# learner-shx/SVG-IR

Hardware: AMD Instinct MI355X
Metric: Gaussian-surfels/sec fwd+bwd @800x800 (1 view) (higher is better)
Workload: dtype f32; 1 GPU; cfg2: rgss path, P=200000 surfels, 800x800, SH degree 3, S=5, VS=0, fwd+bwd, one view per step per GPU (BASELINE.json configs[1] = cfg2 at N=1; configs[3] = cfg4, view r on rank r, at N>1); num_rendered=673008, parallelism=view-parallel x1, per_rank_cpus=not pinned

## Files before the change

svg-ir_amd/csrc/api.hip:

```cpp
#include <algorithm>
#include <cstdarg>
#include <cstdio>
#include <atomic>
#include <cstdlib>
#include <ctime>
#include <memory>
#include <mutex>
#include <string>
#include <vector>

#include "common.hpp"
#include "workload_history.hpp"

using namespace svgir;

namespace {

thread_local std::string g_err;
std::atomic<bool> g_prof{false};
WorkloadHistory g_history;
unsigned long long* pinned_words(size_t n) {
    void* ptr = nullptr;
    if (hipHostMalloc(&ptr, n * sizeof(unsigned long long), hipHostMallocCoherent) != hipSuccess) { (void)hipGetLastError(); return nullptr; }
    std::fill_n((unsigned long long*)ptr, n, 0ull);
    return (unsigned long long*)ptr;
}
unsigned long long* g_pinned = nullptr;
std::atomic<uint32_t> g_pinned_tag{0};
constexpr unsigned kPinnedSlots = 256;
std::once_flag g_pinned_once;
std::mutex g_pinned_mu;
uint64_t g_pinned_busy[kPinnedSlots / 64];
struct PinnedSlot {
    unsigned long long* at = nullptr; uint32_t tag = 0; int index = -1;
    PinnedSlot() {
        std::call_once(g_pinned_once, [] { g_pinned = pinned_words(2 * kPinnedSlots); });
        tag = ++g_pinned_tag;
        if (tag == 0) tag = ++g_pinned_tag;
        if (!g_pinned) return;
        static const unsigned usable = [] { const char* e = getenv("SVGIR_PINNED_SLOTS"); return e ? (unsigned)std::min<long>(std::max<long>(atol(e), 0), kPinnedSlots) : kPinnedSlots; }();
        std::lock_guard<std::mutex> lk(g_pinned_mu);
        for (unsigned i = 0; i < usable; i++)
            if (!(g_pinned_busy[i / 64] >> (i % 64) & 1ull)) {
                g_pinned_busy[i / 64] |= 1ull << (i % 64);
                index = (int)i;
                at = g_pinned + 2 * index;
                return;
            }
    }
    ~PinnedSlot() {
        if (index < 0) return;
        std::lock_guard<std::mutex> lk(g_pinned_mu);
        g_pinned_busy[index / 64] &= ~(1ull << (index % 64));
    }
    PinnedSlot(const PinnedSlot&) = delete;
    PinnedSlot& operator=(const PinnedSlot&) = delete;
};
double spin_budget_s() {
    static const double v = [] {
        const char* e = getenv("SVGIR_SPIN_MS");
        return e ? std::max(0.0, atof(e)) * 1e-3 : 0.05;
    }();
    return v;
}
inline bool tagged_pair(volatile unsigned long long* at, uint32_t tag, uint32_t* w0, uint32_t* w1) {
    const unsigned long long v0 = at[0], v1 = at[1];
    if ((uint32_t)(v0 >> 32) != tag || (uint32_t)(v1 >> 32) != tag) return false;
    *w0 = (uint32_t)v0; *w1 = (uint32_t)v1;
    return true;
}
bool pinned_spin(volatile unsigned long long* at, uint32_t tag, uint32_t* w0, uint32_t* w1) {
    struct timespec t0;
    clock_gettime(CLOCK_MONOTONIC, &t0);
    const double budget = spin_budget_s();
    for (long long spin = 0;; spin++) {
        if (tagged_pair(at, tag, w0, w1)) return true;
        if ((spin & 255) == 255 || budget == 0.0) {
            struct timespec t1;
            clock_gettime(CLOCK_MONOTONIC, &t1);
            const double el = (double)(t1.tv_sec - t0.tv_sec) + 1e-9 * (double)(t1.tv_nsec - t0.tv_nsec);
            if (el >= budget) return false;
            if (el > 5e-3) { struct timespec ts = {0, 20000}; nanosleep(&ts, nullptr); }
        }
    }
}
struct ViewEntry { const void* key = nullptr; uint32_t tag = 0; int cap_R = 0; long long cap_slots = -1; unsigned long long stamp = 0;
                   bool queue = false;
                   bool recorded = false;
                   hipStream_t stream = nullptr; };
constexpr int kViewEntries = 1024;
std::mutex g_view_mu;
ViewEntry g_view[kViewEntries];
constexpr int kViewWords = 4;
unsigned long long* g_view_pinned = nullptr;
unsigned long long g_view_clock = 0;
// ... 394 lines not shown
            if (int rc = check("prepass")) return rc;
            if (timed) stage_mark(tm, "prepass");
        }
        if (p->shade) {
            svgir_shade_params sp = p->shade->sp;
            sp.subset = nullptr; sp.subset_count = nullptr;
            if (prepass) {
                uint32_t* cnt = G.shade_work + partition_work_words(P) - 1;
                launch_partition(P, G.needed, nullptr, G.shade_list, G.shade_work, cnt, s);
                sp.subset = G.shade_list; sp.subset_count = cnt;
            } else if (shade_subset) {
                sp.subset = depth_order; sp.subset_count = G.counters + 3;
            }
            if (shade_forward_impl(&sp, p->shade->reduced, const_cast<float*>(p->features), const_cast<float*>(p->vfeatures), true, s) != 0)
                return fail(SVGIR_ERR_INVALID, "fused shading: svgir_shade_forward rejected its parameters");
            if (int rc = check("shade")) return rc;
            if (timed) stage_mark(tm, "shade");
        }
        if (features_ready && hipStreamWaitEvent(s, features_ready, 0) != hipSuccess) return fail(SVGIR_ERR_HIP, "waiting for the features event");
        if (launch_render_fwd(ra, svgss, s) < 0) launch_render_fwd_generic(ra, svgss, s);
        if (int rc = check("render")) return rc;
        if (timed) stage_mark(tm, "render");
        return 0;
    }

    int begin() {
        if (int rc = validate(p, true)) return rc;
        features_ready = (hipEvent_t)p->features_ready;
        if (!o || !c.geom || !c.binning || !c.image) return fail(SVGIR_ERR_INVALID, "outputs / allocators must be provided");
        P = p->P; v = view_grid(p->W, p->H);
        svgss = p->variant == SVGIR_SVGSS;
        if (P == 0) {
            const size_t N = (size_t)v.W * v.H;
            HIP_OK(hipMemsetAsync(o->out_color, 0, 3 * N * 4, s));
            HIP_OK(hipMemsetAsync(o->out_normal, 0, 3 * N * 4, s));
            HIP_OK(hipMemsetAsync(o->out_depth, 0, N * 4, s));
            HIP_OK(hipMemsetAsync(o->out_opacity, 0, N * 4, s));
            if (p->S) HIP_OK(hipMemsetAsync(o->out_feature, 0, (size_t)p->S * N * 4, s));
            if (svgss && p->VS) HIP_OK(hipMemsetAsync(o->out_vfeature, 0, (size_t)(p->VS / 4) * N * 4, s));
            if (!svgss && o->out_pseudo_normal) HIP_OK(hipMemsetAsync(o->out_pseudo_normal, 0, 3 * N * 4, s));
            if (!svgss && o->out_surface_xyz) HIP_OK(hipMemsetAsync(o->out_surface_xyz, 0, 3 * N * 4, s));
            done = true;
            return 1;
        }
        gblob = c.geom(geom_layout(nullptr, P).bytes, c.geom_ctx);
        iblob = c.image(image_layout(nullptr, v.W, v.H).bytes, c.image_ctx);
        if (!gblob || !iblob) return fail(SVGIR_ERR_ALLOC, "geometry/image blob allocation failed");
        G = geom_layout(gblob, P);
        I = image_layout(iblob, v.W, v.H);

        PreArgs pa;
        camera_args(pa, p);
        pa.W = v.W; pa.H = v.H; pa.gx = v.gx; pa.gy = v.gy; pa.colors_precomp = p->colors_precomp; pa.opacities = p->opacities;
        pa.cov3D_precomp = p->cov3D_precomp; pa.patchbbox = p->patchbbox;
        pa.rec = G.rec; pa.cov3D = G.cov3D; pa.clamped = G.clamped; pa.tiles = G.tiles; pa.key = G.key[0]; pa.idx = G.idx[0];
        pa.radii = o->radii;
        pa.out_weights = o->out_weights;
        pa.features = nullptr; pa.embed_S = 0;
        if (rec_embeds_features(p->S, svgss ? p->VS : 0)) {
            if (features_ready && hipStreamWaitEvent(s, features_ready, 0) != hipSuccess) return fail(SVGIR_ERR_HIP, "waiting for the features event");
            features_ready = nullptr; pa.features = p->features; pa.embed_S = p->S; }
        shade_subset = p->shade && !p->shade->all_surfels;
        prepass = shade_subset && shade_prepass(p->shade->sp.Ns);
        pa.needed = prepass ? G.needed : nullptr;
        pa.span = G.counters + 3;
        if (p->shade) pa.tabs = shade_tables(&p->shade->sp, nullptr, 0);
        pa.zero_words = radix_gtot(G.radix_tbl, P); pa.n_zero_words = (int)radix_gtot_words(P);
        ckey = workload_key(p);
        static const bool key_spec_env = getenv("SVGIR_NO_KEY_SPEC") == nullptr;
        spec_top = (key_spec && key_spec_env) ? g_history.guess_top(ckey) : -1;
        pa.spec_top = spec_top; pa.key_top = G.key_top;
        pa.prefilter_violation = nullptr;
        if (p->prefiltered) {
            HIP_OK(hipMemsetAsync(G.counters, 0, 16, s));
            pa.prefilter_violation = G.counters + 1;
        }
        launch_preprocess(pa, svgss, s);
        if (int rc = check("preprocess")) return rc;
        stage_mark(tm, "preprocess");

        const int depth_bits = spec_top >= 0 ? 24 : 32;
        depth_order = G.idx[(depth_bits / 8) & 1];
        const RadixWeights rw{G.tiles, G.radix_wtbl, G.offsets, G.counters, G.key_top, (P + 63) / 64, pa.prefilter_violation, R_pin.at, R_pin.tag};
        launch_radix_sort(G.key, G.idx, P, nullptr, depth_bits, 8, G.radix_tbl, s, &rw);
        if (int rc = check("depth sort")) return rc;
        stage_mark(tm, "sort_depth");

        nstate = seg_nstate(p->S, svgss ? p->VS : 0);
        plan = tile_sort_plan(v.T);
        fin = plan.passes & 1;

        cap = 0; cap_slots = -1; bblob = nullptr;
        CapKey pkey = ckey;
        (void)resolve_view(g_history.last_view(ckey, &pkey.P), nullptr, Wait::kLook, nullptr, false, &pkey);
        long long gs = -1;
        if (const int guess = g_history.guess(ckey, &gs)) {
            cap = binning_capacity((long long)guess + guess / 8 + 1024);
            cap_slots = p->forward_only ? 0 : (gs < 0 ? -1 : std::min<long long>(gs + gs / 8 + 64, (long long)seg_capacity(cap, v.T)));
            bblob = c.binning(bin_layout(nullptr, cap, v.T, nstate, cap_slots).bytes, c.binning_ctx);
            if (bblob) {
                if (int rc = run_binning_and_render(bblob, cap, cap_slots, true)) return rc;
            } else {
                cap = 0;
            }
        }
        return 0;
    }

    static int run(const svgir_view_call& c, bool key_spec) {
        ForwardCall f(c, key_spec);
        const int rc = f.begin();
        return rc != 0 ? (rc < 0 ? rc : 0) : f.finish();
    }

    int finish() {
        if (done) return 0;
        done = true;
        uint32_t R_host = 0, R_aux = 0;
        bool have_R = R_pin.at && pinned_spin(R_pin.at, R_pin.tag, &R_host, &R_aux);
        if (!have_R) {
            const hipError_t e = hipStreamSynchronize(s);
            if (e != hipSuccess) return fail(SVGIR_ERR_HIP, "the forward failed on the device: %s", hipGetErrorString(e));
            have_R = R_pin.at && tagged_pair(R_pin.at, R_pin.tag, &R_host, &R_aux);
            if (!have_R) {
                uint32_t w[3] = {0, 0, 0};
                HIP_OK(hipMemcpy(w, G.counters, 12, hipMemcpyDeviceToHost));
                R_host = w[0]; R_aux = ((p->prefiltered && w[1]) ? 1u << 16 : 0u) | (w[2] & 0xffffu);
            }
        }
        if (p->prefiltered && (R_aux >> 16) != 0u) {
            (void)hipStreamSynchronize(s);
            return fail(SVGIR_ERR_INVALID, "Point is filtered although prefiltered is set. This shouldn't happen!");
        }
        if (R_host > 0x7ffff000u) return fail(SVGIR_ERR_INVALID, "instance count %u overflows int32", R_host);
        const int R = (int)R_host;
        {
            const uint32_t summary = R_aux & 0xffffu;
            if (key_spec) { g_history.record_top(ckey, summary); g_history.count(WorkloadHistory::kForwards); }
            if (spec_top >= 0) g_history.count(WorkloadHistory::kThreePass);
            const int av = (int)((summary >> 8) & 0xffu), ov = (int)(summary & 0xffu);
            if (spec_top >= 0 && !(av == 0xff && ov == 0) && (av != spec_top || ov != spec_top)) {
                HIP_OK(hipStreamSynchronize(s));
                g_history.count(WorkloadHistory::kRerunTop);
                return run(c, false);
            }
        }
        g_history.record_R(ckey, R);
        if (!bblob || R > cap) {
            const bool redo = bblob != nullptr;
            if (redo) { HIP_OK(hipStreamSynchronize(s)); g_history.count(WorkloadHistory::kRerunR); }
            cap = binning_capacity(R);
            cap_slots = p->forward_only ? 0 : -1;
            if (cap_slots < 0 && R > 0) {
                void* tmp = nullptr;
                if (hipMallocAsync(&tmp, bin_layout(nullptr, cap, v.T, nstate, 0).bytes, s) == hipSuccess) {
                    const int rc = run_binning_and_render((char*)tmp, cap, 0, false, true);
                    const ViewCounts vc = rc == 0 ? resolve_view(iblob, nullptr, Wait::kBlock, &s) : ViewCounts{};
                    (void)hipFreeAsync(tmp, s);
                    if (rc) return rc;
                    if (vc.slots >= 0) cap_slots = std::min<long long>(vc.slots, (long long)seg_capacity(cap, v.T));
                } else {
                    (void)hipGetLastError();
                }
            }
            bblob = c.binning(bin_layout(nullptr, cap, v.T, nstate, cap_slots).bytes, c.binning_ctx);
            if (!bblob) return fail(SVGIR_ERR_ALLOC, "binning blob allocation failed");
            if (redo && o->out_weights) HIP_OK(hipMemsetAsync(o->out_weights, 0, (size_t)P * 4, s));
// ... 322 lines not shown
```

svg-ir_amd/csrc/binning.hip:

```cpp
#include <algorithm>
#include <cassert>

#include "common.hpp"

namespace svgir {

namespace {

constexpr int GS = 32;

__device__ __forceinline__ uint32_t key_top_fold(uint32_t a, uint32_t b) { return (a & b & 0xff00u) | ((a | b) & 0xffu); }

struct WeightArgs {
    const uint32_t* vals;
    uint32_t* wgtot;
    RadixWeights w;
};

template <int ITEMS, bool W = false>
__global__ void __launch_bounds__(BLOCK) radix_hist_kernel(const uint32_t* __restrict__ keys, int n_cap,
                                                           const uint32_t* __restrict__ n_dev, int bit_lo,
                                                           uint32_t mask, uint32_t* __restrict__ table,
                                                           uint32_t* __restrict__ gtot, WeightArgs wa) {
    __shared__ uint32_t hist[256];
    __shared__ uint32_t whist[W ? 256 : 1];
    const int n = n_dev ? (int)min((uint32_t)n_cap, n_dev[0]) : n_cap;
    hist[threadIdx.x] = 0;
    if constexpr (W) whist[threadIdx.x] = 0;
    __syncthreads();
    const int base = blockIdx.x * (BLOCK * ITEMS);
    uint32_t k[ITEMS];
#pragma unroll
    for (int i = 0; i < ITEMS; i++) k[i] = keys[max(0, min(base + i * BLOCK + (int)threadIdx.x, n - 1))];
    uint32_t w[W ? ITEMS : 1];
    if constexpr (W) {
        uint32_t g[ITEMS];
#pragma unroll
        for (int i = 0; i < ITEMS; i++) g[i] = wa.vals[max(0, min(base + i * BLOCK + (int)threadIdx.x, n - 1))];
#pragma unroll
        for (int i = 0; i < ITEMS; i++) w[i] = wa.w.tiles[2 * (size_t)g[i]];
    }
#pragma unroll
    for (int i = 0; i < ITEMS; i++) {
        const int e = base + i * BLOCK + threadIdx.x;
        if (e < n) atomicAdd(&hist[(k[i] >> bit_lo) & mask], 1u);
        if constexpr (W) if (e < n && w[i] != 0u) atomicAdd(&whist[(k[i] >> bit_lo) & mask], w[i]);
    }
    __syncthreads();
    const uint32_t c = hist[threadIdx.x];
    table[(size_t)blockIdx.x * 256 + threadIdx.x] = c;
    if (c) atomicAdd(&gtot[(size_t)(blockIdx.x / GS) * 256 + threadIdx.x], c);
    if constexpr (W) {
        const uint32_t wc = whist[threadIdx.x];
        wa.w.wtable[(size_t)blockIdx.x * 256 + threadIdx.x] = wc;
        if (wc) atomicAdd(&wa.wgtot[(size_t)(blockIdx.x / GS) * 256 + threadIdx.x], wc);
    }
}

template <int ITEMS, bool W = false>
__global__ void __launch_bounds__(BLOCK) radix_scatter_kernel(const uint32_t* __restrict__ kin,
                                                              const uint32_t* __restrict__ vin,
                                                              uint32_t* __restrict__ kout, uint32_t* __restrict__ vout,
                                                              int n_cap, const uint32_t* __restrict__ n_dev, int bit_lo, int nbits,
                                                              const uint32_t* __restrict__ table,
                                                              const uint32_t* __restrict__ gtot, int ngroups, WeightArgs wa) {
    __shared__ uint32_t wcnt[4][256];
    __shared__ uint32_t wtot[4];
    __shared__ uint32_t wtot2[W ? 4 : 1], ksum[W ? 4 : 1], smax[W ? 4 : 1];
    const int t = threadIdx.x, lane = t & 63, wave = t >> 6;
    const uint32_t mask = (1u << nbits) - 1;
    const int n = n_dev ? (int)min((uint32_t)n_cap, n_dev[0]) : n_cap;
    const int base = blockIdx.x * (BLOCK * ITEMS) + wave * (64 * ITEMS);
    const unsigned long long lt_mask = (lane == 0) ? 0ull : (~0ull >> (64 - lane));
    uint32_t ks[ITEMS], vs[ITEMS], rk[ITEMS];
#pragma unroll
    for (int c = 0; c < ITEMS; c++) {
        const int e = base + c * 64 + lane;
        ks[c] = e < n ? kin[e] : 0u;
        vs[c] = e < n ? vin[e] : 0u;
    }
    uint32_t ws[W ? ITEMS : 1];
    if constexpr (W) {
#pragma unroll
        for (int c = 0; c < ITEMS; c++) ws[c] = base + c * 64 + lane < n ? wa.w.tiles[2 * (size_t)vs[c]] : 0u;
        if (blockIdx.x == 0) {
            uint32_t kv = 0xff00u;
#pragma unroll 8
            for (int j = t; j < wa.w.n_key_top; j += BLOCK) kv = key_top_fold(kv, wa.w.key_top[j]);
            kv = wave_reduce(kv, key_top_fold);
            if (lane == 0) ksum[wave] = kv;
        }
    }
#pragma unroll
    for (int w = 0; w < 4; w++) wcnt[w][t] = 0;
    uint32_t cursor;
    uint32_t wcursor = 0;
    {
        const int g = blockIdx.x / GS;
        uint32_t tot = 0, pre = 0, wsum = 0, wpre = 0;
#pragma unroll 8
        for (int gg = 0; gg < ngroups; gg++) {
            const uint32_t v = gtot[(size_t)gg * 256 + t];
            tot += v;
            pre += gg < g ? v : 0u;
            if constexpr (W) {
                const uint32_t wv = wa.wgtot[(size_t)gg * 256 + t];
                wsum += wv;
                wpre += gg < g ? wv : 0u;
            }
        }
#pragma unroll 8
        for (int b = g * GS; b < (int)blockIdx.x; b++) {
            pre += table[(size_t)b * 256 + t];
            if constexpr (W) wpre += wa.w.wtable[(size_t)b * 256 + t];
        }
        cursor = block_excl_scan<4>(tot, wtot) + pre;
        if constexpr (W) {
            uint32_t R;
            wcursor = block_excl_scan<4>(wsum, wtot2, &R) + wpre;
            if (blockIdx.x == 0 && t == 0) {
                const uint32_t summary = key_top_fold(key_top_fold(ksum[0], ksum[1]), key_top_fold(ksum[2], ksum[3]));
                wa.w.counters[0] = R;
                wa.w.counters[2] = summary;
                if (wa.w.host_out) {
                    const uint32_t viol = wa.w.violation ? (wa.w.violation[0] != 0u ? 1u : 0u) : 0u;
                    __hip_atomic_store(wa.w.host_out, ((unsigned long long)wa.w.host_tag << 32) | R, __ATOMIC_RELAXED, __HIP_MEMORY_SCOPE_SYSTEM);
                    __hip_atomic_store(wa.w.host_out + 1, ((unsigned long long)wa.w.host_tag << 32) | (viol << 16) | summary, __ATOMIC_RELAXED,
                                       __HIP_MEMORY_SCOPE_SYSTEM);
                }
            }
        }
    }
#pragma unroll
    for (int c = 0; c < ITEMS; c++) {
        const bool valid = base + c * 64 + lane < n;
        const uint32_t d = (ks[c] >> bit_lo) & mask;
        const unsigned long long same = wave_match(d, nbits, valid);
// ... 22 lines not shown
                sV[lp] = vs[c]; sS[lp] = ws[c]; sD[lp] = (uint8_t)d;
                if (ws[c] != 0u) span = max(span, gcur[d] + (lp - bstart[d]) + 1u);
            }
        }
        span = wave_reduce_max(span);
        if (lane == 0) smax[wave] = span;
        __syncthreads();
        const int nblk = min(BLOCK * ITEMS, n - (int)blockIdx.x * (BLOCK * ITEMS));
        uint32_t wv[ITEMS], sum = 0;
#pragma unroll
        for (int c = 0; c < ITEMS; c += 4) {
            const uint4 q = reinterpret_cast<const uint4*>(sS)[(t * ITEMS + c) >> 2];
            wv[c] = q.x; wv[c + 1] = q.y; wv[c + 2] = q.z; wv[c + 3] = q.w;
        }
#pragma unroll
        for (int c = 0; c < ITEMS; c++) { wv[c] = t * ITEMS + c < nblk ? wv[c] : 0u; sum += wv[c]; }
        uint32_t run = block_excl_scan<4>(sum, wtot2);
#pragma unroll
        for (int c = 0; c < ITEMS; c += 4) {
            uint4 q;
            q.x = run; run += wv[c]; q.y = run; run += wv[c + 1]; q.z = run; run += wv[c + 2]; q.w = run; run += wv[c + 3];
            reinterpret_cast<uint4*>(sS)[(t * ITEMS + c) >> 2] = q;
        }
        if (t == 0) {
            const uint32_t m = max(max(smax[0], smax[1]), max(smax[2], smax[3]));
            if (m != 0u) atomicMax(wa.w.counters + 3, m);
        }
        __syncthreads();
#pragma unroll
        for (int c = 0; c < ITEMS; c++) {
            const int i = c * BLOCK + t;
            if (i < nblk) {
                const uint32_t d = sD[i], b = bstart[d];
                const uint32_t pos = gcur[d] + ((uint32_t)i - b);
                vout[pos] = sV[i];
                wa.w.offsets[pos] = wgcur[d] + (sS[i] - sS[b]);
            }
        }
        return;
    }
    if (ITEMS >= 16) {
        __shared__ uint32_t sK[BLOCK * (ITEMS >= 16 ? ITEMS : 1)], sV[BLOCK * (ITEMS >= 16 ? ITEMS : 1)];
        __shared__ uint32_t bstart[256], gcur[256];
        const uint32_t c0 = wcnt[0][t], c1 = wcnt[1][t], c2 = wcnt[2][t], c3 = wcnt[3][t];
        const uint32_t bc = c0 + c1 + c2 + c3;
        const uint32_t bs = block_excl_scan<4>(bc, wtot);
        bstart[t] = bs; gcur[t] = cursor;
        wcnt[0][t] = bs; wcnt[1][t] = bs + c0; wcnt[2][t] = bs + c0 + c1; wcnt[3][t] = bs + c0 + c1 + c2;
        __syncthreads();
#pragma unroll
        for (int c = 0; c < ITEMS; c++) {
            if (base + c * 64 + lane < n) {
                const uint32_t lp = wcnt[wave][(ks[c] >> bit_lo) & mask] + rk[c];
                sK[lp] = ks[c]; sV[lp] = vs[c];
            }
        }
        __syncthreads();
        const int nblk = min(BLOCK * ITEMS, n - (int)blockIdx.x * (BLOCK * ITEMS));
#pragma unroll
        for (int c = 0; c < ITEMS; c++) {
            const int i = c * BLOCK + t;
            if (i < nblk) {
                const uint32_t k = sK[i], d = (k >> bit_lo) & mask;
                const uint32_t pos = gcur[d] + ((uint32_t)i - bstart[d]);
                kout[pos] = k;
                vout[pos] = sV[i];
            }
        }
        return;
    }
    {
        const uint32_t c0 = wcnt[0][t], c1 = wcnt[1][t], c2 = wcnt[2][t];
        __syncthreads();
        wcnt[0][t] = cursor; wcnt[1][t] = cursor + c0; wcnt[2][t] = cursor + c0 + c1; wcnt[3][t] = cursor + c0 + c1 + c2;
    }
    __syncthreads();
#pragma unroll
    for (int c = 0; c < ITEMS; c++) {
        if (base + c * 64 + lane < n) {
            const uint32_t pos = wcnt[wave][(ks[c] >> bit_lo) & mask] + rk[c];
            kout[pos] = ks[c];
            vout[pos] = vs[c];
        }
    }
}

__global__ void __launch_bounds__(BLOCK) ts12_hist_kernel(const uint32_t* __restrict__ keys, int n_cap, const uint32_t* __restrict__ n_dev,
                                                          uint32_t* __restrict__ table, int nbins) {
    __shared__ uint32_t hist[TS12_BINS];
    const int n = n_dev ? (int)min((uint32_t)n_cap, n_dev[0]) : n_cap;
    const int t = threadIdx.x;
    for (int i = t; i < nbins; i += BLOCK) hist[i] = 0u;
    __syncthreads();
    const int base = blockIdx.x * TS12_KEYS;
    uint32_t k[TS12_KEYS / BLOCK];
#pragma unroll
    for (int i = 0; i < TS12_KEYS / BLOCK; i++) k[i] = keys[max(0, min(base + i * BLOCK + t, n - 1))];
#pragma unroll
    for (int i = 0; i < TS12_KEYS / BLOCK; i++)
        if (base + i * BLOCK + t < n) atomicAdd(&hist[k[i] & (TS12_BINS - 1)], 1u);
    __syncthreads();
    uint32_t* row = table + (size_t)blockIdx.x * nbins;
    for (int i = t; i < nbins; i += BLOCK) row[i] = hist[i];
}

__global__ void __launch_bounds__(BLOCK) ts12_colscan_kernel(uint32_t* __restrict__ table, int nb, uint32_t* __restrict__ totals, int nbins) {
    __shared__ uint32_t psum[16][17];
    const int col = threadIdx.x & 15, seg = threadIdx.x >> 4;
    const int d = blockIdx.x * 16 + col;
    const int rps = (nb + 15) / 16, r0 = min(nb, seg * rps), r1 = min(nb, r0 + rps);
    uint32_t* colp = table + d;
    uint32_t sum = 0;
    int r = r0;
    for (; r + 8 <= r1; r += 8) {
        uint32_t c[8];
#pragma unroll
        for (int j = 0; j < 8; j++) c[j] = colp[(size_t)(r + j) * nbins];
#pragma unroll
        for (int j = 0; j < 8; j++) sum += c[j];
    }
    for (; r < r1; r++) sum += colp[(size_t)r * nbins];
    psum[seg][col] = sum;
    __syncthreads();
    uint32_t run = 0, all = 0;
#pragma unroll
    for (int sg = 0; sg < 16; sg++) { const uint32_t v = psum[sg][col]; run += sg < seg ? v : 0u; all += v; }
    if (seg == 0) totals[d] = all;
    r = r0;
    for (; r + 8 <= r1; r += 8) {
        uint32_t c[8];
#pragma unroll
        for (int j = 0; j < 8; j++) c[j] = colp[(size_t)(r + j) * nbins];
#pragma unroll
        for (int j = 0; j < 8; j++) { colp[(size_t)(r + j) * nbins] = run; run += c[j]; }
    }
    for (; r < r1; r++) { const uint32_t c = colp[(size_t)r * nbins]; colp[(size_t)r * nbins] = run; run += c; }
}

__global__ void __launch_bounds__(BLOCK) ts12_scatter_kernel(const uint32_t* __restrict__ kin, const uint32_t* __restrict__ vin,
                                                             uint32_t* __restrict__ kout, uint32_t* __restrict__ vout, int n_cap,
                                                             const uint32_t* __restrict__ n_dev, const uint32_t* __restrict__ table,
                                                             const uint32_t* __restrict__ totals, uint32_t* __restrict__ ranges, int T, int nbins) {
    __shared__ uint32_t cur[TS12_BINS];
    __shared__ uint16_t wcnt[4][TS12_BINS];
    __shared__ uint32_t wtot[4];
    constexpr int PERMAX = TS12_BINS / BLOCK;
    constexpr int ROUNDS = TS12_KEYS / BLOCK;
    const int per = nbins / BLOCK;
    const int t = threadIdx.x, lane = t & 63, wave = t >> 6;
    const int n = n_dev ? (int)min((uint32_t)n_cap, n_dev[0]) : n_cap;
    const int base = blockIdx.x * TS12_KEYS + wave * (64 * ROUNDS);
    const unsigned long long lt_mask = (lane == 0) ? 0ull : (~0ull >> (64 - lane));
    uint32_t ks[ROUNDS], vs[ROUNDS];
    uint16_t rk[ROUNDS];
#pragma unroll
    for (int c = 0; c < ROUNDS; c++) {
        const int e = base + c * 64 + lane;
        ks[c] = e < n ? kin[e] : 0u;
        vs[c] = e < n ? vin[e] : 0u;
    }
    uint32_t tot[PERMAX], pre[PERMAX];
    {
        const uint32_t* tp = totals + t * per;
        const uint32_t* rp = table + (size_t)blockIdx.x * nbins + t * per;
#pragma unroll
        for (int j = 0; j < PERMAX; j++) { tot[j] = j < per ? tp[j] : 0u; pre[j] = j < per ? rp[j] : 0u; }
// ... 140 lines not shown
    unsigned long long run = 0;
    uint32_t n_empty = 0;
#pragma unroll
    for (int w = 0; w < 16; w++) { run += wsum2[w]; n_empty += wzero[w]; }
    uint32_t n_mine;
    hist[t] = block_excl_scan<16>(hist[t], wsum, &n_mine);
    __syncthreads();
    for (int i0 = p0; i0 < p1; i0 += 1024) {
        const int i = i0 + t;
        const unsigned long long v = both(i < p1 ? counts[i] : 0u);
        const unsigned long long inc = (unsigned long long)wave_incl_scan_u32((uint32_t)v) | ((unsigned long long)wave_incl_scan_u32((uint32_t)(v >> 32)) << 32);
        __syncthreads();
        unsigned long long all;
        const unsigned long long ex = run + block_excl_scan<16>(v, inc, wsum2, &all);
        if (i < p1) {
            if (prefix) prefix[i] = (uint32_t)ex;
            if (slot_prefix) slot_prefix[i] = (uint32_t)(ex >> 32);
        }
        run += all;
    }
    if (c == 7 && t == 0) {
        if (total) {
            total[1] = (uint32_t)run; total[2] = (uint32_t)(run >> 32);
            total[3] = magic; total[4] = cap_R; total[5] = (uint32_t)(unsigned long long)cap_slots; total[6] = (uint32_t)((unsigned long long)cap_slots >> 32);
        }
        if (host_total) {
            __hip_atomic_store(host_total + 2, ((unsigned long long)host_tag << 32) | (unsigned long long)((uint32_t)n - n_empty), __ATOMIC_RELAXED, __HIP_MEMORY_SCOPE_SYSTEM);
            __hip_atomic_store(host_total, ((unsigned long long)host_tag << 32) | (run & 0xffffffffull), __ATOMIC_RELAXED, __HIP_MEMORY_SCOPE_SYSTEM);
            __hip_atomic_store(host_total + 1, ((unsigned long long)host_tag << 32) | (run >> 32), __ATOMIC_RELAXED, __HIP_MEMORY_SCOPE_SYSTEM);
        }
    }
    for (int i = t; i < n; i += 1024) {
        const int tile = i >> 2;
        if (xcd_of_tile(tile % gx, tile / gx) != c) continue;
        const uint32_t len = counts[i];
        order[8u * atomicAdd(&hist[1023u - min(1023u, len)], 1u) + c] = (uint32_t)i;
    }
    for (uint32_t j = n_mine + (uint32_t)t; 8u * j + c < (uint32_t)order_n; j += 1024u) order[8u * j + c] = ORDER_NONE;
}

}

void launch_order_desc(const uint32_t* counts, int n, uint32_t* order, uint32_t* prefix, uint32_t* slot_prefix, uint32_t* totals,
                       unsigned long long* host_totals, uint32_t host_tag, uint32_t cap_R, long long cap_slots, uint32_t magic, int gx, int order_n,
                       hipStream_t s) {
    hipLaunchKernelGGL(order_xcd_kernel, dim3(8), dim3(1024), 0, s, counts, n, order, prefix, slot_prefix, totals, host_totals,
                       host_tag, cap_R, cap_slots, magic, gx, order_n);
}

template <int ITEMS>
static void radix_sort_impl(uint32_t* const key[2], uint32_t* const val[2], int n, const uint32_t* n_dev, int total_bits,
                            int bits_per_pass, uint32_t* tbl, uint32_t* gtot, hipStream_t s, const RadixWeights* weights) {
    const int per = BLOCK * ITEMS;
    const int nb = (n + per - 1) / per;
    const int ng = (nb + GS - 1) / GS;
    const int passes = (total_bits + bits_per_pass - 1) / bits_per_pass;
    assert(!weights || (n_dev == nullptr && bits_per_pass <= 8 && passes <= RADIX_WGTOT_SLOT));
    for (int p = 0; p < passes; p++) {
        const int lo = p * bits_per_pass, nbits = std::min(bits_per_pass, total_bits - lo);
        uint32_t* gt = gtot + (size_t)p * ng * 256;
        if (weights && p == passes - 1) {
            const WeightArgs wa{val[p & 1], gtot + (size_t)RADIX_WGTOT_SLOT * ng * 256, *weights};
            hipLaunchKernelGGL((radix_hist_kernel<ITEMS, true>), dim3(nb), dim3(BLOCK), 0, s, key[p & 1], n, n_dev, lo,
                               (1u << nbits) - 1, tbl, gt, wa);
            hipLaunchKernelGGL((radix_scatter_kernel<ITEMS, true>), dim3(nb), dim3(BLOCK), 0, s, key[p & 1], val[p & 1],
                               key[(p + 1) & 1], val[(p + 1) & 1], n, n_dev, lo, nbits, tbl, gt, ng, wa);
            break;
        }
        hipLaunchKernelGGL((radix_hist_kernel<ITEMS>), dim3(nb), dim3(BLOCK), 0, s, key[p & 1], n, n_dev, lo,
                           (1u << nbits) - 1, tbl, gt, WeightArgs{});
        hipLaunchKernelGGL((radix_scatter_kernel<ITEMS>), dim3(nb), dim3(BLOCK), 0, s, key[p & 1], val[p & 1],
                           key[(p + 1) & 1], val[(p + 1) & 1], n, n_dev, lo, nbits, tbl, gt, ng, WeightArgs{});
    }
}

void launch_radix_sort(uint32_t* const key[2], uint32_t* const val[2], int n, const uint32_t* n_dev, int total_bits,
                       int bits_per_pass, uint32_t* table, hipStream_t s, const RadixWeights* weights) {
    if (n <= 0) return;
    uint32_t* gtot = radix_gtot(table, n);
    if (n <= (1 << 20)) radix_sort_impl<4>(key, val, n, n_dev, total_bits, bits_per_pass, table, gtot, s, weights);
    else radix_sort_impl<16>(key, val, n, n_dev, total_bits, bits_per_pass, table, gtot, s, weights);
}

void launch_emit(int P, const uint32_t* order, const uint32_t* tiles, const uint32_t* offsets, float* rec,
                 const int32_t* radii, int gx, int gy, uint32_t* tile_keys, uint32_t* vals, int cap, uint32_t* ranges,
                 uint32_t* seg_count, uint32_t* sort_table, const uint32_t* span, uint32_t* disp_ctr, hipStream_t s) {
    hipLaunchKernelGGL(emit_kernel, dim3((P + BLOCK - 1) / BLOCK), dim3(BLOCK), 0, s, P, order, tiles, offsets, rec,
                       radii, gx, gy, tile_keys, vals, (uint32_t)cap, ranges, 2 * gx * gy + (gx * gy + 255) / 256 * SEG_BLOCK_STRIDE, seg_count,
                       radix_gtot(sort_table, cap), (int)radix_gtot_words(cap), span, disp_ctr);
}

void launch_tile_sort12(uint32_t* const key[2], uint32_t* const val[2], int n, const uint32_t* n_dev, uint32_t* table, uint32_t* ranges, int T,
                        hipStream_t s) {
    if (n <= 0) return;
    const int nb = (n + TS12_KEYS - 1) / TS12_KEYS;
    const int nbins = (T + BLOCK - 1) / BLOCK * BLOCK;
    uint32_t* totals = table + (size_t)nb * nbins;
    hipLaunchKernelGGL(ts12_hist_kernel, dim3(nb), dim3(BLOCK), 0, s, key[0], n, n_dev, table, nbins);
    hipLaunchKernelGGL(ts12_colscan_kernel, dim3(nbins / 16), dim3(BLOCK), 0, s, table, nb, totals, nbins);
    hipLaunchKernelGGL(ts12_scatter_kernel, dim3(nb), dim3(BLOCK), 0, s, key[0], val[0], key[1], val[1], n, n_dev, table, totals, ranges, T, nbins);
}

void launch_ranges(int R, const uint32_t* R_dev, const uint32_t* tile_keys, uint32_t* ranges, int T, hipStream_t s) {
    if (R > 0) hipLaunchKernelGGL(ranges_kernel, dim3((R + BLOCK - 1) / BLOCK), dim3(BLOCK), 0, s, R, R_dev, tile_keys, ranges);
}

}
```

Measured before the change: 582.3 million surfels/s.

## Replace LSD depth radix sort with MSD bucket scatter plus per-bucket block sort

When the key-top guess is available and P is at most 2^19, the depth sort now makes one global MSD pass on the top byte. That pass scatters only visible surfels and compacts culled ones to the tail. Then one 1024-thread workgroup per bucket finishes sorting in shared memory, or in global memory for oversized buckets, and computes the tile-offset prefix sums inline. This is meant to replace the multi-pass 24-bit LSD radix sort (three histogram+scatter pairs) with about three launches, and to skip sorting culled surfels. It adds a large shared-memory kernel with limited occupancy, and it risks load imbalance when depth buckets are skewed.

```diff
diff --git a/svg-ir_amd/csrc/api.hip b/svg-ir_amd/csrc/api.hip
--- a/svg-ir_amd/csrc/api.hip
+++ b/svg-ir_amd/csrc/api.hip
@@ -11,6 +11,7 @@
 
 #include "common.hpp"
 #include "workload_history.hpp"
+#include "depth_sort_plan.hpp"
 
 using namespace svgir;
 
@@ -571,7 +572,10 @@
         const int depth_bits = spec_top >= 0 ? 24 : 32;
         depth_order = G.idx[(depth_bits / 8) & 1];
         const RadixWeights rw{G.tiles, G.radix_wtbl, G.offsets, G.counters, G.key_top, (P + 63) / 64, pa.prefilter_violation, R_pin.at, R_pin.tag};
-        launch_radix_sort(G.key, G.idx, P, nullptr, depth_bits, 8, G.radix_tbl, s, &rw);
+        static const bool forced_lsd = depth_sort_forced_lsd(getenv("SVGIR_DEPTH_SORT"));
+        static const int bucket_cap = depth_bucket_cap(getenv("SVGIR_DEPTH_BUCKET_CAP"));
+        if (depth_sort_plan(P, spec_top, forced_lsd) == DepthSortPlan::kBuckets) launch_depth_bucket_sort(G.key, G.idx, P, G.radix_tbl, bucket_cap, s, rw);
+        else launch_radix_sort(G.key, G.idx, P, nullptr, depth_bits, 8, G.radix_tbl, s, &rw);
         if (int rc = check("depth sort")) return rc;
         stage_mark(tm, "sort_depth");
 
diff --git a/svg-ir_amd/csrc/binning.hip b/svg-ir_amd/csrc/binning.hip
--- a/svg-ir_amd/csrc/binning.hip
+++ b/svg-ir_amd/csrc/binning.hip
@@ -2,6 +2,7 @@
 #include <cassert>
 
 #include "common.hpp"
+#include "depth_sort_plan.hpp"
 
 namespace svgir {
 
@@ -17,7 +18,7 @@
     RadixWeights w;
 };
 
-template <int ITEMS, bool W = false>
+template <int ITEMS, bool W = false, bool F = false>
 __global__ void __launch_bounds__(BLOCK) radix_hist_kernel(const uint32_t* __restrict__ keys, int n_cap,
                                                            const uint32_t* __restrict__ n_dev, int bit_lo,
                                                            uint32_t mask, uint32_t* __restrict__ table,
@@ -43,7 +44,8 @@
 #pragma unroll
     for (int i = 0; i < ITEMS; i++) {
         const int e = base + i * BLOCK + threadIdx.x;
-        if (e < n) atomicAdd(&hist[(k[i] >> bit_lo) & mask], 1u);
+        if constexpr (F) { if (e < n && w[i] != 0u) atomicAdd(&hist[(k[i] >> bit_lo) & mask], 1u); }
+        else if (e < n) atomicAdd(&hist[(k[i] >> bit_lo) & mask], 1u);
         if constexpr (W) if (e < n && w[i] != 0u) atomicAdd(&whist[(k[i] >> bit_lo) & mask], w[i]);
     }
     __syncthreads();
@@ -52,7 +54,7 @@
     if (c) atomicAdd(&gtot[(size_t)(blockIdx.x / GS) * 256 + threadIdx.x], c);
     if constexpr (W) {
         const uint32_t wc = whist[threadIdx.x];
-        wa.w.wtable[(size_t)blockIdx.x * 256 + threadIdx.x] = wc;
+        if constexpr (!F) wa.w.wtable[(size_t)blockIdx.x * 256 + threadIdx.x] = wc;
         if (wc) atomicAdd(&wa.wgtot[(size_t)(blockIdx.x / GS) * 256 + threadIdx.x], wc);
     }
 }
@@ -241,6 +243,251 @@
             kout[pos] = ks[c];
             vout[pos] = vs[c];
         }
+    }
+}
+
+
+template <int ITEMS>
+__global__ void __launch_bounds__(BLOCK) depth_bucket_scatter_kernel(const uint32_t* __restrict__ kin, const uint32_t* __restrict__ vin,
+                                                                     uint32_t* __restrict__ kout, uint32_t* __restrict__ vout,
+                                                                     uint32_t* __restrict__ wout, int n, int bit_lo,
+                                                                     const uint32_t* __restrict__ table, const uint32_t* __restrict__ gtot,
+                                                                     const uint32_t* __restrict__ wgtot, int ngroups, RadixWeights w) {
+    __shared__ uint32_t wcnt[4][256];
+    __shared__ uint32_t wtot[4], wtot2[4], wtot3[4], ksum[4], wcul[4];
+    const int t = threadIdx.x, lane = t & 63, wave = t >> 6;
+    const int base = blockIdx.x * (BLOCK * ITEMS) + wave * (64 * ITEMS);
+    const unsigned long long lt_mask = (lane == 0) ? 0ull : (~0ull >> (64 - lane));
+    uint32_t ks[ITEMS], vs[ITEMS], ws[ITEMS], rk[ITEMS];
+#pragma unroll
+    for (int c = 0; c < ITEMS; c++) {
+        const int e = base + c * 64 + lane;
+        ks[c] = e < n ? kin[e] : 0u;
+        vs[c] = e < n ? vin[e] : 0u;
+    }
+#pragma unroll
+    for (int c = 0; c < ITEMS; c++) ws[c] = base + c * 64 + lane < n ? w.tiles[2 * (size_t)vs[c]] : 0u;
+    if (blockIdx.x == 0) {
+        uint32_t kv = 0xff00u;
+#pragma unroll 8
+        for (int j = t; j < w.n_key_top; j += BLOCK) kv = key_top_fold(kv, w.key_top[j]);
+        kv = wave_reduce(kv, key_top_fold);
+        if (lane == 0) ksum[wave] = kv;
+    }
+#pragma unroll
+    for (int q = 0; q < 4; q++) wcnt[q][t] = 0;
+    uint32_t cursor, nvis, cull_base;
+    {
+        const int g = blockIdx.x / GS;
+        uint32_t tot = 0, pre = 0, wsum = 0;
+#pragma unroll 8
+        for (int gg = 0; gg < ngroups; gg++) {
+            const uint32_t v = gtot[(size_t)gg * 256 + t];
+            tot += v;
+            pre += gg < g ? v : 0u;
+            if (blockIdx.x == 0) wsum += wgtot[(size_t)gg * 256 + t];
+        }
+#pragma unroll 8
+        for (int b = g * GS; b < (int)blockIdx.x; b++) pre += table[(size_t)b * 256 + t];
+        cursor = block_excl_scan<4>(tot, wtot, &nvis) + pre;
+        cull_base = nvis + blockIdx.x * (BLOCK * ITEMS) - block_sum<4>(pre, wtot3);
+        if (blockIdx.x == 0) {
+            uint32_t R;
+            (void)block_excl_scan<4>(wsum, wtot2, &R);
+            if (t == 0) {
+                const uint32_t summary = key_top_fold(key_top_fold(ksum[0], ksum[1]), key_top_fold(ksum[2], ksum[3]));
+                w.counters[0] = R;
+                w.counters[2] = summary;
+                w.counters[3] = nvis;
+                if (w.host_out) {
+                    const uint32_t viol = w.violation ? (w.violation[0] != 0u ? 1u : 0u) : 0u;
+                    __hip_atomic_store(w.host_out, ((unsigned long long)w.host_tag << 32) | R, __ATOMIC_RELAXED, __HIP_MEMORY_SCOPE_SYSTEM);
+                    __hip_atomic_store(w.host_out + 1, ((unsigned long long)w.host_tag << 32) | (viol << 16) | summary, __ATOMIC_RELAXED,
+                                       __HIP_MEMORY_SCOPE_SYSTEM);
+                }
+            }
+        }
+    }
+    uint32_t ncul = 0;
+#pragma unroll
+    for (int c = 0; c < ITEMS; c++) {
+        const bool valid = base + c * 64 + lane < n && ws[c] != 0u;
+        const uint32_t d = (ks[c] >> bit_lo) & 255u;
+        const unsigned long long same = wave_match(d, 8, valid);
+        const uint32_t in_round = (uint32_t)__popcll(same & lt_mask);
+        const uint32_t prior = wcnt[wave][d];
+        rk[c] = prior + in_round;
+        if (valid && in_round == 0) wcnt[wave][d] = prior + (uint32_t)__popcll(same);
+        const unsigned long long culled = __ballot(base + c * 64 + lane < n && ws[c] == 0u);
+        if (!valid) rk[c] = ncul + (uint32_t)__popcll(culled & lt_mask);
+        ncul += (uint32_t)__popcll(culled);
+    }
+    if (lane == 0) wcul[wave] = ncul;
+    __syncthreads();
+    {
+        const uint32_t c0 = wcnt[0][t], c1 = wcnt[1][t], c2 = wcnt[2][t];
+        __syncthreads();
+        wcnt[0][t] = cursor; wcnt[1][t] = cursor + c0; wcnt[2][t] = cursor + c0 + c1; wcnt[3][t] = cursor + c0 + c1 + c2;
+    }
+    __syncthreads();
+    for (int q = 0; q < wave; q++) cull_base += wcul[q];
+#pragma unroll
+    for (int c = 0; c < ITEMS; c++) {
+        if (base + c * 64 + lane >= n) continue;
+        if (ws[c] != 0u) {
+            const uint32_t pos = wcnt[wave][(ks[c] >> bit_lo) & 255u] + rk[c];
+            kout[pos] = ks[c];
+            vout[pos] = vs[c];
+            wout[pos] = ws[c];
+        } else {
+            vout[cull_base + rk[c]] = vs[c];
+        }
+    }
+}
+
+constexpr int DB_THREADS = 1024, DB_WAVES = DB_THREADS / 64, DB_ROUNDS = DEPTH_BUCKET_CAP / DB_THREADS;
+
+template <bool CARRY, class Get, class Put>
+__device__ __forceinline__ void bucket_pass(int m, int shift, Get get, Put put, uint32_t (*wcnt)[256], uint32_t* cur, uint32_t* wsum) {
+    const int t = threadIdx.x, lane = t & 63, wave = t >> 6;
+    const unsigned long long lt_mask = (lane == 0) ? 0ull : (~0ull >> (64 - lane));
+    for (int i = t; i < DB_WAVES * 256; i += DB_THREADS) (&wcnt[0][0])[i] = 0u;
+    __syncthreads();
+    const int per = ((m + DB_WAVES - 1) / DB_WAVES + 63) & ~63;
+    const int base = wave * per;
+    uint2 it[DB_ROUNDS];
+    uint32_t rk[DB_ROUNDS];
+#pragma unroll
+    for (int r = 0; r < DB_ROUNDS; r++) {
+        if (r * 64 < per) {
+            const int i = base + r * 64 + lane;
+            const bool valid = i < m;
+            it[r] = valid ? get(i) : make_uint2(0u, 0u);
+            const uint32_t d = (it[r].x >> shift) & 255u;
+            const unsigned long long same = wave_match(d, 8, valid);
+            const uint32_t in_round = (uint32_t)__popcll(same & lt_mask);
+            const uint32_t prior = wcnt[wave][d];
+            rk[r] = prior + in_round;
+            if (valid && in_round == 0) wcnt[wave][d] = prior + (uint32_t)__popcll(same);
+        }
+    }
+    __syncthreads();
+    uint32_t c[DB_WAVES], total = 0;
+#pragma unroll
+    for (int q = 0; q < DB_WAVES; q++) { c[q] = t < 256 ? wcnt[q][t] : 0u; total += c[q]; }
+    uint32_t run;
+    if constexpr (CARRY) run = t < 256 ? cur[t] : 0u;
+    else run = block_excl_scan<DB_WAVES>(total, wsum);
+    if (t < 256) {
+#pragma unroll
+        for (int q = 0; q < DB_WAVES; q++) { wcnt[q][t] = run; run += c[q]; }
+        if constexpr (CARRY) cur[t] = run;
+    }
+    __syncthreads();
+#pragma unroll
+    for (int r = 0; r < DB_ROUNDS; r++) {
+        if (r * 64 < per) {
+            const int i = base + r * 64 + lane;
+            if (i < m) put(wcnt[wave][(it[r].x >> shift) & 255u] + rk[r], it[r]);
+        }
+    }
+    __syncthreads();
+}
+
+__global__ void __launch_bounds__(DB_THREADS) depth_bucket_sort_kernel(uint32_t* key0, uint32_t* val0, uint32_t* key1, uint32_t* val1, uint32_t* offsets,
+                                                                       const uint32_t* __restrict__ tiles, const uint32_t* __restrict__ gtot,
+                                                                       const uint32_t* __restrict__ wgtot, int ngroups, int cap) {
+    __shared__ uint32_t sA[DEPTH_BUCKET_CAP], sB[DEPTH_BUCKET_CAP], sI[DEPTH_BUCKET_CAP], sW[DEPTH_BUCKET_CAP];
+    __shared__ uint32_t wcnt[DB_WAVES][256];
+    __shared__ uint32_t cur[256], wsum[DB_WAVES], wsum2[DB_WAVES], hdr[3], red[2][DB_WAVES];
+    const int t = threadIdx.x, lane = t & 63, wave = t >> 6;
+    uint32_t cnt = 0, wt = 0;
+    if (t < 256)
+        for (int g = 0; g < ngroups; g++) { cnt += gtot[(size_t)g * 256 + t]; wt += wgtot[(size_t)g * 256 + t]; }
+    const uint32_t cpre = block_excl_scan<DB_WAVES>(cnt, wsum);
+    const uint32_t wpre = block_excl_scan<DB_WAVES>(wt, wsum2);
+    if (t == (int)blockIdx.x) { hdr[0] = cpre; hdr[1] = cnt; hdr[2] = wpre; }
+    __syncthreads();
+    const uint32_t start = hdr[0], wbase = hdr[2];
+    const int n = (int)hdr[1];
+    if (n == 0) return;
+    if (n <= cap) {
+        for (int i = t; i < n; i += DB_THREADS) {
+            sA[i] = (key1[start + i] << 16) | (uint32_t)i;
+            sI[i] = val1[start + i];
+            sW[i] = offsets[start + i];
+        }
+        bucket_pass<false>(n, 16, [&](int i) { return make_uint2(sA[i], 0u); }, [&](uint32_t pos, uint2 it) { sB[pos] = it.x; }, wcnt, cur, wsum);
+        bucket_pass<false>(n, 24, [&](int i) { return make_uint2(sB[i], 0u); }, [&](uint32_t pos, uint2 it) { sA[pos] = it.x; }, wcnt, cur, wsum);
+        uint32_t wv[DB_ROUNDS], sum = 0;
+#pragma unroll
+        for (int j = 0; j < DB_ROUNDS; j++) {
+            const int i = t * DB_ROUNDS + j;
+            wv[j] = i < n ? sW[sA[i] & 0xffffu] : 0u;
+            sum += wv[j];
+        }
+        uint32_t run = block_excl_scan<DB_WAVES>(sum, wsum2);
+#pragma unroll
+        for (int j = 0; j < DB_ROUNDS; j++) {
+            const int i = t * DB_ROUNDS + j;
+            if (i < n) sB[i] = run;
+            run += wv[j];
+        }
+        __syncthreads();
+        for (int i = t; i < n; i += DB_THREADS) {
+            val1[start + i] = sI[sA[i] & 0xffffu];
+            offsets[start + i] = wbase + sB[i];
+        }
+        return;
+    }
+    {
+        uint32_t a = 0xffffu, o = 0u;
+        for (int i = t; i < n; i += DB_THREADS) { const uint32_t k = key1[start + i] & 0xffffu; a &= k; o |= k; }
+        a = wave_reduce(a, [](uint32_t x, uint32_t y) { return x & y; });
+        o = wave_reduce(o, [](uint32_t x, uint32_t y) { return x | y; });
+        if (lane == 0) { red[0][wave] = a; red[1][wave] = o; }
+        __syncthreads();
+        a = 0xffffu; o = 0u;
+#pragma unroll
+        for (int q = 0; q < DB_WAVES; q++) { a &= red[0][q]; o |= red[1][q]; }
+        if (a != o) {
+            for (int pass = 0; pass < 2; pass++) {
+                const uint32_t* sk = (pass ? key0 : key1) + start; const uint32_t* sv = (pass ? val0 : val1) + start;
+                uint32_t* dk = (pass ? key1 : key0) + start; uint32_t* dv = (pass ? val1 : val0) + start;
+                const int shift = 8 * pass;
+                if (t < 256) cur[t] = 0u;
+                __syncthreads();
+                for (int i = t; i < n; i += DB_THREADS) atomicAdd(&cur[(sk[i] >> shift) & 255u], 1u);
+                __syncthreads();
+                const uint32_t ex = block_excl_scan<DB_WAVES>(t < 256 ? cur[t] : 0u, wsum);
+                if (t < 256) cur[t] = ex;
+                for (int c0 = 0; c0 < n; c0 += cap)
+                    bucket_pass<true>(min(cap, n - c0), shift, [&](int i) { return make_uint2(sk[c0 + i], sv[c0 + i]); },
+                                      [&](uint32_t pos, uint2 it) { dk[pos] = it.x; dv[pos] = it.y; }, wcnt, cur, wsum);
+                __threadfence_block();
+                __syncthreads();
+            }
+        }
+    }
+    uint32_t carry = wbase;
+    for (int c0 = 0; c0 < n; c0 += DB_THREADS * DB_ROUNDS) {
+        uint32_t wv[DB_ROUNDS], sum = 0;
+#pragma unroll
+        for (int j = 0; j < DB_ROUNDS; j++) {
+            const int i = c0 + t * DB_ROUNDS + j;
+            wv[j] = i < n ? tiles[2 * (size_t)val1[start + i]] : 0u;
+            sum += wv[j];
+        }
+        uint32_t all;
+        uint32_t run = carry + block_excl_scan<DB_WAVES>(sum, wsum, &all);
+#pragma unroll
+        for (int j = 0; j < DB_ROUNDS; j++) {
+            const int i = c0 + t * DB_ROUNDS + j;
+            if (i < n) offsets[start + i] = run;
+            run += wv[j];
+        }
+        carry += all;
+        __syncthreads();
     }
 }
 
@@ -547,6 +794,20 @@
     else radix_sort_impl<16>(key, val, n, n_dev, total_bits, bits_per_pass, table, gtot, s, weights);
 }
 
+void launch_depth_bucket_sort(uint32_t* const key[2], uint32_t* const val[2], int n, uint32_t* table, int cap, hipStream_t s, const RadixWeights& w) {
+    if (n <= 0) return;
+    constexpr int ITEMS = 4;
+    assert(n <= DEPTH_BUCKET_MAX_P && cap >= DEPTH_BUCKET_CAP_MIN && cap <= DEPTH_BUCKET_CAP);
+    const int nb = (n + BLOCK * ITEMS - 1) / (BLOCK * ITEMS), ng = (nb + GS - 1) / GS;
+    uint32_t* gtot = radix_gtot(table, n);
+    uint32_t* wgtot = gtot + (size_t)RADIX_WGTOT_SLOT * ng * 256;
+    const WeightArgs wa{val[0], wgtot, w};
+    hipLaunchKernelGGL((radix_hist_kernel<ITEMS, true, true>), dim3(nb), dim3(BLOCK), 0, s, key[0], n, (const uint32_t*)nullptr, 16, 255u, table, gtot, wa);
+    hipLaunchKernelGGL((depth_bucket_scatter_kernel<ITEMS>), dim3(nb), dim3(BLOCK), 0, s, key[0], val[0], key[1], val[1], w.offsets, n, 16, table, gtot,
+                       wgtot, ng, w);
+    hipLaunchKernelGGL(depth_bucket_sort_kernel, dim3(256), dim3(DB_THREADS), 0, s, key[0], val[0], key[1], val[1], w.offsets, w.tiles, gtot, wgtot, ng, cap);
+}
+
 void launch_emit(int P, const uint32_t* order, const uint32_t* tiles, const uint32_t* offsets, float* rec,
                  const int32_t* radii, int gx, int gy, uint32_t* tile_keys, uint32_t* vals, int cap, uint32_t* ranges,
                  uint32_t* seg_count, uint32_t* sort_table, const uint32_t* span, uint32_t* disp_ctr, hipStream_t s) {
diff --git a/svg-ir_amd/csrc/depth_sort_plan.hpp b/svg-ir_amd/csrc/depth_sort_plan.hpp
--- /dev/null
+++ b/svg-ir_amd/csrc/depth_sort_plan.hpp
@@ -0,0 +1,28 @@
+#pragma once
+#include <cstdlib>
+#include <cstring>
+
+namespace svgir {
+
+enum class DepthSortPlan { kLsd = 0, kBuckets = 1 };
+
+constexpr int DEPTH_BUCKET_MAX_P = 1 << 19;
+constexpr int DEPTH_BUCKET_CAP = 8192;
+constexpr int DEPTH_BUCKET_CAP_MIN = 64;
+
+inline bool depth_sort_forced_lsd(const char* env) { return env && std::strcmp(env, "lsd") == 0; }
+inline int depth_bucket_cap(const char* env) {
+    if (!env || !env[0]) return DEPTH_BUCKET_CAP;
+    const long v = std::strtol(env, nullptr, 10);
+    return v < DEPTH_BUCKET_CAP_MIN ? DEPTH_BUCKET_CAP_MIN : (v > DEPTH_BUCKET_CAP ? DEPTH_BUCKET_CAP : (int)v);
+}
+
+inline DepthSortPlan depth_sort_plan(int P, int spec_top, bool forced_lsd) {
+    return (!forced_lsd && spec_top >= 0 && P > 0 && P <= DEPTH_BUCKET_MAX_P) ? DepthSortPlan::kBuckets : DepthSortPlan::kLsd;
+}
+
+#if defined(__HIPCC__)
+void launch_depth_bucket_sort(uint32_t* const key[2], uint32_t* const val[2], int n, uint32_t* table, int cap, hipStream_t s, const RadixWeights& w);
+#endif
+
+}
```

Result: faster. 608.9 million surfels/s (median of 6 runs) (+4.6%).
